# Wu0409/DuPL

Measured on AMD Instinct MI355X. Metric: training img/s at 448^2, VOC dual-student ViT-B/16, phase B step, higher is better.
Workload: dtype f32 storage / accumulation / results; Linear GEMMs (forward, dgrad, wgrad), attention (forward, backward) and the decoder convs as fp32-equivalent f16x3 split products on the f16 MFMA (operands as fp16 hi / lo planes, 3 products per block, fp32 accumulate; error vs fp64 <= the f32 MFMA kernels'); CA

## Files before the change

dupl_amd/csrc/attn_split_bwd.hip:

```cpp
#include "common.h"
#include "../../include/dupl_hip.h"

namespace {

typedef _Float16 h8 __attribute__((ext_vector_type(8)));
typedef _Float16 h4 __attribute__((ext_vector_type(4)));
constexpr float LO_INV = 1.f / DUPL_LO_SCALE;
constexpr int HD = 64, TT = 32;
constexpr int PL = 4096;
constexpr int MAXN = 2048;

#define MFMA16(a, b, c) __builtin_amdgcn_mfma_f32_32x32x16_f16((a), (b), (c), 0, 0, 0)

__device__ __forceinline__ float fast_exp(float x) { return __builtin_amdgcn_exp2f(x * 1.4426950408889634f); }

__device__ __forceinline__ void xcd_remap3(int remap, int& bx, int& by, int& bz) {
    bx = blockIdx.x; by = blockIdx.y; bz = blockIdx.z;
    if (!remap) return;
    const int gx = gridDim.x, gy = gridDim.y;
    const int total = gx * gy * gridDim.z;
    const int L = bx + gx * (by + gy * bz);
    const int q = total >> 3, r = total & 7;
    const int xcd = L & 7, idx = L >> 3;
    const int w = (xcd < r ? xcd * (q + 1) : r * (q + 1) + (xcd - r) * q) + idx;
// ... 67 lines not shown
}

__global__ __launch_bounds__(256) void delta_kernel(const float* __restrict__ out, const float* __restrict__ dout,
                                                    float* __restrict__ delta, int B, int N, int H) {
    const long idx = (long)blockIdx.x * blockDim.x + threadIdx.x;
    const long total = (long)B * N * H;
    if (idx >= total) return;
    const int h = (int)(idx % H);
    const long bn = idx / H;
    const int n = (int)(bn % N), b = (int)(bn / N);
    const float4* o = reinterpret_cast<const float4*>(out + bn * (long)(H * HD) + h * HD);
    const float4* d = reinterpret_cast<const float4*>(dout + bn * (long)(H * HD) + h * HD);
    float s = 0.f;
#pragma unroll
    for (int i = 0; i < HD / 4; ++i) {
        const float4 a = o[i], c = d[i];
        s += (a.x * c.x + a.y * c.y) + (a.z * c.z + a.w * c.w);
    }
    delta[((long)b * H + h) * N + n] = s;
}

__device__ __forceinline__ void attn_bwd16_dq_body(char* __restrict__ smem, const int bx, const int h, const int b,
                                                   const __half* __restrict__ qkv_hi, const __half* __restrict__ qkv_lo,
                                                   const __half* __restrict__ do_hi, const __half* __restrict__ do_lo,
                                                   const float* __restrict__ lse, const float* __restrict__ delta,
                                                   const float* __restrict__ slot, float* __restrict__ dqkv, unsigned int* __restrict__ amax_out, int N, int H,
                                                   float scale) {
    constexpr int STAGE = 6 * PL;
    const int tid = threadIdx.x, lane = tid & 63, wave = tid >> 6, l31 = lane & 31, hf = lane >> 5;
    const int q0 = bx * 128 + wave * 32;
    const int D = H * HD, ld = 3 * D;
    const int qrow = q0 + l31;
// ... 278 lines not shown
    }
    const int bx = w % gx, h = (w / gx) % H, b = w / (gx * H);
    if (role == 0) attn_bwd16_dkv_body<1>(smem, bx, h, b, qkv_hi, qkv_lo, do_hi, do_lo, lse, delta, slot, dqkv, amax_out, N, H, scale);
    else if (role == 1) attn_bwd16_dq_body(smem, bx, h, b, qkv_hi, qkv_lo, do_hi, do_lo, lse, delta, slot, dqkv, amax_out, N, H, scale);
    else attn_bwd16_dkv_body<0>(smem, bx, h, b, qkv_hi, qkv_lo, do_hi, do_lo, lse, delta, slot, dqkv, amax_out, N, H, scale);
}

}

constexpr int g_attnb16_remap = 1;

extern "C" int dupl_attention_bwd16(const void* qkv_hi, const void* qkv_lo, const float* out, const float* dout, const void* do_hi,
                                    const void* do_lo, const float* do_slot, const float* lse, float* delta, float* dqkv, int32_t B,
                                    int32_t N, int32_t H, int32_t hd, float scale, void* amax_out, dupl_stream_t stream) {
    unsigned int* ax = static_cast<unsigned int*>(amax_out);
    if (!qkv_hi || !qkv_lo || !out || !dout || !do_hi || !do_lo || !do_slot || !lse || !delta || !dqkv || B <= 0 || N <= 0 ||
        N > MAXN || H <= 0 || hd != HD)
        return DUPL_ERR_ARG;
    hipStream_t s = (hipStream_t)stream;
    const long total = (long)B * N * H;
    DUPL_LAUNCH(delta_kernel, dim3((unsigned)((total + 255) / 256)), dim3(256), 0, s, out, dout, delta, B, N, H);
    const unsigned blocks = 3u * (unsigned)(((N + 127) / 128) * H * B);
    DUPL_LAUNCH(attn_bwd16_all_kernel, dim3(blocks), dim3(256), 0, s, (const __half*)qkv_hi, (const __half*)qkv_lo,
                       (const __half*)do_hi, (const __half*)do_lo, lse, delta, do_slot, dqkv, ax, N, H, B, scale, g_attnb16_remap);
    return dupl_launch_status();
}
```

dupl_amd/csrc/common.h:

```cpp
#pragma once
#include <hip/hip_runtime.h>
#include <hip/hip_fp16.h>
#include <stdint.h>

#define DUPL_OK 0
#define DUPL_ERR_ARG (-1)
#define DUPL_ERR_LAUNCH (-2)

#define DUPL_WAVE 64


typedef float f32x4 __attribute__((ext_vector_type(4)));
typedef float f32x16 __attribute__((ext_vector_type(16)));

#include <tuple>
#include <utility>
static thread_local int dupl_tl_launch_err = DUPL_OK;

template <typename... KArgs, typename... Args, size_t... I>
static inline hipError_t dupl_launch_impl(void (*kernel)(KArgs...), dim3 grid, dim3 block, size_t shmem, hipStream_t stream,
                                          std::index_sequence<I...>, Args&&... args) {
    std::tuple<KArgs...> vals{static_cast<KArgs>(std::forward<Args>(args))...};
    void* ptrs[sizeof...(KArgs) ? sizeof...(KArgs) : 1] = {static_cast<void*>(&std::get<I>(vals))...};
    return hipLaunchKernel(reinterpret_cast<const void*>(kernel), grid, block, ptrs, shmem, stream);
// ... 21 lines not shown
}
__device__ __forceinline__ float bil_scale(int in, int out, bool align) {
    if (align) return out > 1 ? (float)(in - 1) / (float)(out - 1) : 0.f;
    return (float)in / (float)out;
}

__device__ __forceinline__ float wave_sum(float v) {
#pragma unroll
    for (int o = 32; o > 0; o >>= 1) v += __shfl_xor(v, o, 64);
    return v;
}
__device__ __forceinline__ float wave_max(float v) {
#pragma unroll
    for (int o = 32; o > 0; o >>= 1) v = fmaxf(v, __shfl_xor(v, o, 64));
    return v;
}
__device__ __forceinline__ float wave_min(float v) {
#pragma unroll
    for (int o = 32; o > 0; o >>= 1) v = fminf(v, __shfl_xor(v, o, 64));
    return v;
}
__device__ __forceinline__ double wave_sum_d(double v) {
#pragma unroll
    for (int o = 32; o > 0; o >>= 1) v += __shfl_xor(v, o, 64);
    return v;
}

__device__ __forceinline__ float block_sum(float v, float* red) {
    v = wave_sum(v);
    const int w = threadIdx.x >> 6, l = threadIdx.x & 63, nw = (blockDim.x + 63) >> 6;
// ... 93 lines not shown
```

dupl_amd/csrc/gemm_split.hip:

```cpp
#include "common.h"
#include <type_traits>
#include "../../include/dupl_hip.h"

#ifndef G16_ABL
#define G16_ABL 0
#endif

namespace {

typedef _Float16 h8 __attribute__((ext_vector_type(8)));

constexpr int TBK = 32;
constexpr float LO_INV = 1.f / DUPL_LO_SCALE;

template <bool F1>
__global__ __launch_bounds__(256) void split_kernel(const float* __restrict__ x, __half* __restrict__ hi, __half* __restrict__ lo,
                                                    long n4, float scale) {
    for (long i = (long)blockIdx.x * blockDim.x + threadIdx.x; i < n4; i += (long)gridDim.x * blockDim.x) {
        const float4 v = reinterpret_cast<const float4*>(x)[i];
        __half h[4], l[4];
        if constexpr (F1) {
            split_f32_u(v.x * scale, h[0], l[0]);
            split_f32_u(v.y * scale, h[1], l[1]);
            split_f32_u(v.z * scale, h[2], l[2]);
// ... 1429 lines not shown
    const int g16_f1_big_from = G16_F1_BIG_FROM;
    auto al16 = [](const void* q) { return (reinterpret_cast<uintptr_t>(q) & 15) == 0; };
    if (!al16(d->A_hi) || !al16(d->A_lo) || !al16(d->B_hi) || !al16(d->B_lo)) return DUPL_ERR_ARG;
    if (!d->C && !d->C_hi) return DUPL_ERR_ARG;
    if ((d->C_hi == nullptr) != (d->C_lo == nullptr)) return DUPL_ERR_ARG;
    if ((d->flags & (DUPL_GEMM_STORE_PRE | DUPL_GEMM_MUL_DGELU | DUPL_GEMM_MUL_RELUMASK)) && !d->aux) return DUPL_ERR_ARG;
    if (d->flags & ~(DUPL_GEMM_GELU | DUPL_GEMM_RELU | DUPL_GEMM_STORE_PRE | DUPL_GEMM_ACCUM | DUPL_GEMM_MUL_DGELU |
                     DUPL_GEMM_MUL_RELUMASK))
        return DUPL_ERR_ARG;
    const bool accum = d->flags & DUPL_GEMM_ACCUM;
    if (accum && (!d->C || d->C_hi || d->bias || d->res || d->c_rows)) return DUPL_ERR_ARG;
    if (d->c_rows < 0 || (d->c_rows && (d->flags & (DUPL_GEMM_MUL_DGELU | DUPL_GEMM_MUL_RELUMASK)))) return DUPL_ERR_ARG;
    if (d->amax_out && (accum || d->c_rows || (reinterpret_cast<uintptr_t>(d->amax_out) & 3))) return DUPL_ERR_ARG;
    const bool kmajor = d->a_layout || d->b_layout;
    if (d->fmt < 0 || d->fmt > 1 || d->out_exp < 0 || d->out_exp > 15 || (d->out_exp && d->fmt != 1) ||
        (d->fmt == 1 && !kmajor && (accum || d->amax_out)))
        return DUPL_ERR_ARG;
    hipStream_t s = (hipStream_t)stream;
    int ksplit = 1;
    if (accum) {
        const long tiles = (long)((d->M + 127) / 128) * ((d->N + 127) / 128);
        ksplit = (int)((512 + tiles - 1) / tiles);
        const int maxs = (d->K / TBK + 7) / 8;
        if (ksplit > maxs) ksplit = maxs;
        if (ksplit < 1) ksplit = 1;
        if (d->deterministic) ksplit = 1;
    }
    int tile = g16_tile;
    if (tile == 0) {
        const long b256 = (long)((d->M + 255) / 256) * ((d->N + 127) / 128);
        const long b128 = (long)((d->M + 127) / 128) * ((d->N + 127) / 128) * ksplit;
// ... 41 lines not shown
            else DUPL_LAUNCH((gemm_f16x3_km_kernel<2, 2, 4, 2, 2, false, 2, true, true>), persist_grid(nb21), dim3(512), 0, s, *d, g16_group_ring);
        } else {
            if (d->a_layout || !d->b_layout) return DUPL_ERR_ARG;
            DUPL_LAUNCH((gemm_f16x3_km_kernel<2, 2, 4, 2, 2, false, 0, false, true>), persist_grid(nb21), dim3(512), 0, s, *d, g16_group_ring);
        }
        return dupl_launch_status();
    }
    if (d->fmt == 1) {
        const int nb22 = ((d->M + 255) / 256) * ((d->N + 255) / 256), nb21 = ((d->M + 255) / 256) * ((d->N + 127) / 128);
        int t = (g16_tile == 8 || g16_tile == 12 || g16_tile == 14) ? g16_tile : (nb22 >= g16_f1_big_from ? 8 : 12);
        if (d->K / TBK < 3 && t == 14) t = 12;
        if (t == 8) {
            const int cn = (d->N + 255) / 256, rm = (d->M + 255) / 256, cus = 256;
            const int full = nb22 / cus, tail = nb22 - full * cus;
            const int r_big = full > 0 ? (full * cus) / cn : 0;
            if (g16_tile == 0 && full > 0 && tail > 0 && tail * 10 < cus * 3 && r_big > 0 && r_big < rm && !d->amax_out) {
                const int M1 = r_big * 256;
                dupl_gemm16_desc d1 = *d, d2 = *d;
                d1.M = M1;
                d2.M = d->M - M1;
                auto adv = [&](const void* q, size_t elems, size_t bytes) { return q ? static_cast<const void*>(static_cast<const char*>(q) + elems * bytes) : nullptr; };
                d2.A_hi = adv(d->A_hi, (size_t)M1 * d->lda, 2); d2.A_lo = adv(d->A_lo, (size_t)M1 * d->lda, 2);
                d2.C = (float*)adv(d->C, (size_t)M1 * d->ldc, 4);
                d2.C_hi = (void*)adv(d->C_hi, (size_t)M1 * d->ldo, 2); d2.C_lo = (void*)adv(d->C_lo, (size_t)M1 * d->ldo, 2);
                d2.res = (const float*)adv(d->res, (size_t)M1 * d->ldr, 4);
                d2.aux = (float*)adv(d->aux, (size_t)M1 * d->ldaux, 4);
                if (d->c_rows > 0) {
                    if (d->c_rows <= M1) {
                        d2.c_rows = 0; d2.C = nullptr; d2.aux = nullptr; d2.flags &= ~DUPL_GEMM_STORE_PRE;
                    } else { d1.c_rows = 0; d2.c_rows = d->c_rows - M1; }
                }
// ... 37 lines not shown
```

dupl_amd/csrc/split_prep.hip:

```cpp
#include "common.h"
#include "../../include/dupl_hip.h"

namespace {

__global__ __launch_bounds__(256) void amax_kernel(const float* __restrict__ x, long n4, unsigned int* __restrict__ out) {
    __shared__ float red[4];
    float m = 0.f;
    for (long i = (long)blockIdx.x * blockDim.x + threadIdx.x; i < n4; i += (long)gridDim.x * blockDim.x) {
        const float4 v = reinterpret_cast<const float4*>(x)[i];
        m = fmaxf(m, fmaxf(fmaxf(fabsf(v.x), fabsf(v.y)), fmaxf(fabsf(v.z), fabsf(v.w))));
    }
    m = wave_max(m);
    if ((threadIdx.x & 63) == 0) red[threadIdx.x >> 6] = m;
    __syncthreads();
    if (threadIdx.x == 0) {
        m = fmaxf(fmaxf(red[0], red[1]), fmaxf(red[2], red[3]));
        if (m > 0.f) atomicMax(out, __float_as_uint(m));
    }
}

__device__ __forceinline__ void scale_from_amax(unsigned int bits, int target, float& s, float& inv) {
    const float a = __uint_as_float(bits);
    s = 1.f;
    inv = 1.f;
    if (a > 0.f && a < INFINITY) {
        int e;
        frexpf(a, &e);
        s = ldexpf(1.f, target - e);
        inv = ldexpf(1.f, e - target);
    }
}

template <bool F1 = false>
__device__ __forceinline__ void split_rt_tile(const float* __restrict__ x, const int ld, const int R, const int C, const float s,
                                              __half* __restrict__ hi, __half* __restrict__ lo, __half* __restrict__ hiT,
                                              __half* __restrict__ loT, const int Rp, float* __restrict__ colsum, const int r0,
                                              const int c0, const int Rz = 0) {
    __shared__ unsigned int tile[64][65];
    __shared__ float csum[4][64];
    const int tid = threadIdx.x;
    float4 cs = make_float4(0.f, 0.f, 0.f, 0.f);
#pragma unroll
    for (int i = 0; i < 4; ++i) {
        const int c = tid + 256 * i;
        const int r = c >> 4, cc = (c & 15) << 2;
        float4 v = make_float4(0.f, 0.f, 0.f, 0.f);
        const bool in = r0 + r < R && c0 + cc < C;
        if (in) v = *reinterpret_cast<const float4*>(x + (size_t)(r0 + r) * ld + c0 + cc);
        cs.x += v.x; cs.y += v.y; cs.z += v.z; cs.w += v.w;
        __half h[4], l[4];
        if constexpr (F1) {
            split_f32_u(v.x * s, h[0], l[0]);
            split_f32_u(v.y * s, h[1], l[1]);
            split_f32_u(v.z * s, h[2], l[2]);
            split_f32_u(v.w * s, h[3], l[3]);
        } else {
            split_f32(v.x * s, h[0], l[0]);
            split_f32(v.y * s, h[1], l[1]);
            split_f32(v.z * s, h[2], l[2]);
            split_f32(v.w * s, h[3], l[3]);
        }
        if (hi && c0 + cc < C && r0 + r < (Rz > R ? Rz : R)) {
            *reinterpret_cast<uint2*>(hi + (size_t)(r0 + r) * C + c0 + cc) = *reinterpret_cast<const uint2*>(h);
            *reinterpret_cast<uint2*>(lo + (size_t)(r0 + r) * C + c0 + cc) = *reinterpret_cast<const uint2*>(l);
// ... 27 lines not shown
        const int col = c >> 3, rr = (c & 7) << 3;
        if (c0 + col >= C || r0 + rr >= Rp) continue;
        unsigned int w[8];
#pragma unroll
        for (int j = 0; j < 8; ++j) w[j] = tile[rr + j][col];
        uint4 oh, ol;
        oh.x = (w[0] & 0xffffu) | (w[1] << 16); oh.y = (w[2] & 0xffffu) | (w[3] << 16);
        oh.z = (w[4] & 0xffffu) | (w[5] << 16); oh.w = (w[6] & 0xffffu) | (w[7] << 16);
        ol.x = (w[0] >> 16) | (w[1] & 0xffff0000u); ol.y = (w[2] >> 16) | (w[3] & 0xffff0000u);
        ol.z = (w[4] >> 16) | (w[5] & 0xffff0000u); ol.w = (w[6] >> 16) | (w[7] & 0xffff0000u);
        *reinterpret_cast<uint4*>(hiT + (size_t)(c0 + col) * Rp + r0 + rr) = oh;
        *reinterpret_cast<uint4*>(loT + (size_t)(c0 + col) * Rp + r0 + rr) = ol;
    }
}

template <bool F1>
__global__ __launch_bounds__(256) void split_rt_kernel(const float* __restrict__ x, int ld, int R, int C, float* __restrict__ slot,
                                                       unsigned int* __restrict__ next_bits, __half* __restrict__ hi,
                                                       __half* __restrict__ lo, __half* __restrict__ hiT, __half* __restrict__ loT,
                                                       int Rp, int target, float* __restrict__ colsum, int Rz) {
    float s = 1.f;
    if (slot) {
        float inv;
        scale_from_amax(reinterpret_cast<const unsigned int*>(slot)[2], target, s, inv);
        if (blockIdx.x == 0 && blockIdx.y == 0 && threadIdx.x == 0) {
            slot[0] = s;
            slot[1] = inv;
            if (next_bits) *next_bits = 0u;
        }
    }
    split_rt_tile<F1>(x, ld, R, C, s, hi, lo, hiT, loT, Rp, colsum, blockIdx.y * 64, blockIdx.x * 64, Rz);
}

struct split_multi_args {
    dupl_split_item it[DUPL_SPLIT_MULTI_MAX];
    int first[DUPL_SPLIT_MULTI_MAX + 1];
    int n;
};
__global__ __launch_bounds__(256) void split_rt_multi_kernel(const split_multi_args a) {
    int i = 0;
#pragma unroll 1
    while (i + 1 < a.n && (int)blockIdx.x >= a.first[i + 1]) ++i;
    const dupl_split_item& d = a.it[i];
    const int t = blockIdx.x - a.first[i];
    const int tx = (d.C + 63) / 64;
    split_rt_tile(d.x, d.ld, d.R, d.C, 1.f, (__half*)d.hi, (__half*)d.lo, (__half*)d.hiT, (__half*)d.loT, d.Rp, nullptr,
                  (t / tx) * 64, (t % tx) * 64);
}

}

extern "C" int dupl_split_prepare_multi(const dupl_split_item* items, int32_t n, dupl_stream_t stream) {
    if (!items || n < 1 || n > DUPL_SPLIT_MULTI_MAX) return DUPL_ERR_ARG;
    split_multi_args a;
    a.n = n;
    int total = 0;
    for (int i = 0; i < n; ++i) {
        const dupl_split_item& d = items[i];
        if (!d.x || d.R <= 0 || d.C <= 0 || (d.C & 3) || (d.ld & 3) || d.ld < d.C || (!d.hi && !d.hiT) ||
            ((d.hi == nullptr) != (d.lo == nullptr)) || ((d.hiT == nullptr) != (d.loT == nullptr)) ||
            (d.hiT && (d.Rp < d.R || (d.Rp & 7))) || (reinterpret_cast<uintptr_t>(d.x) & 15))
            return DUPL_ERR_ARG;
        a.it[i] = d;
        a.first[i] = total;
        const int Rt = d.hiT ? d.Rp : d.R;
        total += ((d.C + 63) / 64) * ((Rt + 63) / 64);
    }
    a.first[n] = total;
    DUPL_LAUNCH(split_rt_multi_kernel, dim3((unsigned)total), dim3(256), 0, (hipStream_t)stream, a);
    return dupl_launch_status();
}

extern "C" int dupl_split_prepare(const dupl_split_desc* d, dupl_stream_t stream) {
    if (!d || d->struct_size != sizeof(dupl_split_desc)) return DUPL_ERR_ARG;
    const float* x = d->x;
    const int ld = d->ld, R = d->R, C = d->C, Rp = d->Rp, target_exp = d->target_exp, amax_mode = d->amax_mode;
    float* slot = d->slot;
    void *hi = d->hi, *lo = d->lo, *hiT = d->hiT, *loT = d->loT;
    if (amax_mode < 0 || amax_mode > 2 || (amax_mode && !slot)) return DUPL_ERR_ARG;
    if (d->colsum_accum && d->deterministic) return DUPL_ERR_ARG;
    if (!x || R <= 0 || C <= 0 || (C & 3) || (ld & 3) || ld < C || (!hi && !hiT) || ((hi == nullptr) != (lo == nullptr)) ||
        ((hiT == nullptr) != (loT == nullptr)) || (hiT && (Rp < R || (Rp & 7))) || target_exp < 1 || target_exp > 15)
        return DUPL_ERR_ARG;
    if (d->fmt < 0 || d->fmt > 1 || d->rows_zero_to < 0 || (d->rows_zero_to && (d->rows_zero_to < R || !hi))) return DUPL_ERR_ARG;
    if ((reinterpret_cast<uintptr_t>(x) & 15)) return DUPL_ERR_ARG;
    hipStream_t s = (hipStream_t)stream;
    if (slot && amax_mode != 1) {
        if (ld != C) return DUPL_ERR_ARG;
        if (amax_mode == 2 && hipMemsetAsync(reinterpret_cast<unsigned int*>(slot) + 2, 0, 4, s) != hipSuccess) return DUPL_ERR_LAUNCH;
        const long n4 = (long)R * C / 4;
        long g = (n4 + 2047) / 2048;
        if (g > 256) g = 256;
        if (g < 1) g = 1;
        DUPL_LAUNCH(amax_kernel, dim3((unsigned)g), dim3(256), 0, s, x, n4, reinterpret_cast<unsigned int*>(slot) + 2);
    }
    int Rt = hiT ? Rp : R;
    if (d->rows_zero_to > Rt) Rt = d->rows_zero_to;
    const dim3 grid((C + 63) / 64, (Rt + 63) / 64);
    if (d->fmt == 1)
        DUPL_LAUNCH(split_rt_kernel<true>, grid, dim3(256), 0, s, x, ld, R, C, slot, (unsigned int*)d->next_bits, (__half*)hi,
                           (__half*)lo, (__half*)hiT, (__half*)loT, Rp, target_exp, d->colsum_accum, d->rows_zero_to);
    else
        DUPL_LAUNCH(split_rt_kernel<false>, grid, dim3(256), 0, s, x, ld, R, C, slot, (unsigned int*)d->next_bits, (__half*)hi,
                           (__half*)lo, (__half*)hiT, (__half*)loT, Rp, target_exp, d->colsum_accum, d->rows_zero_to);
    return dupl_launch_status();
}
```

dupl_amd/engine.py:

```python
from __future__ import annotations

import os
from dataclasses import dataclass, field
from typing import Dict, List, Optional, Tuple

import torch

from . import ops

Tensor = torch.Tensor

GEMM_MODE = os.environ.get("DUPL_GEMM", "f16x3")


def set_gemm_mode(mode: str):
    global GEMM_MODE
    assert mode in ("f32", "f16x3"), mode
    GEMM_MODE = mode


@dataclass(frozen=True)
class EncoderConfig:
    embed_dim: int = 768
    depth: int = 12
# ... 55 lines not shown
def param_segment(key: str) -> int:
    if key in ("encoder.pos_embed", "encoder.head.weight", "encoder.head.bias"):
        return SEG_FROZEN
    if key.startswith("encoder."):
        return SEG_NORM if "norm" in key[len("encoder."):] else SEG_BACKBONE
    if key.startswith("decoder."):
        return SEG_DECODER
    return SEG_CLS


FMT1 = os.environ.get("DUPL_FMT1", "1") != "0"
KM_BWD = os.environ.get("DUPL_KM_BWD", "1") != "0"
SK_DGRAD = os.environ.get("DUPL_SK_DGRAD", "1") != "0"
WGRAD_GROUP = os.environ.get("DUPL_WGRAD_GROUP", "1") != "0"

SK_DGRAD_MAX_COLS = 1024
ZERO_WS = os.environ.get("DUPL_ZERO_WS", "1") != "0"
FUSED_PLANES = os.environ.get("DUPL_ADAMW_PLANES", "1") != "0"
MERGED_PASS = int(os.environ.get("DUPL_MERGED_PASS", "16384"))
ATTN_SEGS = int(os.environ.get("DUPL_ATTN_SEGS", "1536"))


class FlatStorage:

    def __init__(self, cfg: EncoderConfig, num_classes: int, n_students: int, device="cpu"):
        self.cfg, self.num_classes, self.n_students = cfg, num_classes, n_students
        shapes = student_param_shapes(cfg, num_classes)
        self.shapes = shapes
        self.layout: Dict[str, Tuple[int, int]] = {}
        self.seg_bounds: List[Tuple[int, int]] = []
# ... 94 lines not shown
        old = self._w16_key[student]
        self._w16_key[student] = key
        self.guard.params_changed(student, rewritten=(old is None or old[0] != key[0] or old[2] != key[2] or old[3] != key[3]),
                                  key=key)

    def w16T(self, student: int, key: str, rows: int):
        ver = self._param_key()
        hit = self._w16T.get((student, key))
        if hit is not None and hit[0] == ver:
            return hit[1]
        w = self.view(student, key).view(rows, -1)
        _, T, _ = ops.split_prepare(w, scaled=False, want_rm=False, want_T=True, rows_pad=rows)
        self._w16T[(student, key)] = (ver, T)
        return T

    def w16T_missing(self, student: int, keys_rows):
        ver = self._param_key()
        out = []
        for key, rows in keys_rows:
            hit = self._w16T.get((student, key))
            if hit is None or hit[0] != ver:
                out.append((key, rows, self.view(student, key).view(rows, -1)))
        return out

    def w16T_put(self, student: int, key: str, T):
        self._w16T[(student, key)] = (self._param_key(), T)

    def w16(self, student: int, key: str, rows: int, fmt1: Optional[bool] = None) -> "ops.W16":
        off, n = self.layout[key]
        base = student * self.student_numel + off
        p = self.data16.data_ptr()
        have = ops.EXP_W if (FMT1 and param_segment(key) == SEG_BACKBONE) else 0
        if fmt1 is None:
            fmt1 = bool(have)
        if bool(have) == bool(fmt1):
            return ops.W16(p + 2 * base, p + 2 * (self.data.numel() + base), rows, n // rows, have)
        assert not fmt1
        ver = self._param_key()
        hit = self._w16F0.get((student, key))
        if hit is None or hit[0] != ver:
            hit = (ver, ops.split16(self.view(student, key).view(rows, -1)))
# ... 217 lines not shown
            self._pos_cache.clear()
            self._pos_version = ver
        key = (h, w)
        if key not in self._pos_cache:
            self._pos_cache[key] = ops.pos_embed_resize(pe, self.cfg.grid, h, w)
        return self._pos_cache[key]

    def mark_grad(self, seg: int):
        self.store.seg_has_grad[self.student][seg] = True

    def w16(self, key: str, rows: int, fmt1: Optional[bool] = None):
        return self.store.w16(self.student, key, rows, fmt1)

    def w16T(self, key: str, rows: int):
        return self.store.w16T(self.student, key, rows)


@dataclass
class BlockSaved:
    x_in: Tensor = None
    mean1: Tensor = None
    rstd1: Tensor = None
    ln1: Tensor = None
    qkv: Tensor = None
    lse: Tensor = None
    att: Tensor = None
    x_mid: Tensor = None
    mean2: Tensor = None
    rstd2: Tensor = None
    ln2: Tensor = None
# ... 442 lines not shown

def _linear_backward16_km(P: StudentParams, dy: Tensor, x16, name: str, dgelu_of: Optional[Tensor] = None,
                          dx_feeds_split: bool = False, wgrads: Optional[list] = None) -> Tensor:
    M, N = dy.shape
    Kp = max(96, (M + 31) // 32 * 32)
    fuse_bias = not ops.deterministic()
    dy16, _, alpha = ops.split_prepare(dy, scaled=True, want_rm=True, want_T=False, fmt1=True, rm_rows=Kp,
                                       colsum_into=P.g[name + ".bias"] if fuse_bias else None)
    gw = P.g[name + ".weight"]
    if wgrads is not None:
        wgrads.append((dy16, x16, gw.view(N, -1), alpha))
    else:
        _lin16(P, dy16, x16, out=gw.view(N, -1), accumulate=True, alpha=alpha, a_kmajor=True, b_kmajor=True, k_pad=Kp)
    if not fuse_bias:
        ops.colsum(dy, P.g[name + ".bias"], accumulate=True)
    W16 = P.w16(name + ".weight", N, True)
    if SK_DGRAD and dgelu_of is None and not dx_feeds_split and not ops.deterministic() and W16.cols <= SK_DGRAD_MAX_COLS:
        dx = ops.zero_workspace(M, W16.cols, dy.device) if ZERO_WS else ops.zeros((M, W16.cols), dy.device)
        _lin16(P, dy16.rows_slice(0, M), W16, out=dx, accumulate=True, alpha=alpha, b_kmajor=True)
        return dx
    dx, _ = _lin16(P, dy16.rows_slice(0, M), W16, alpha=alpha, dgelu_of=dgelu_of, amax_for_next=dx_feeds_split, b_kmajor=True)
    return dx


def _linear_backward16(P: StudentParams, dy: Tensor, x: Tensor, name: str, dgelu_of: Optional[Tensor] = None,
                       has_bias: bool = True, dx_feeds_split: bool = False, xT16=None) -> Tensor:
    M, N = dy.shape
    Mp = (M + 31) // 32 * 32
    fuse_bias = has_bias and not ops.deterministic()
    dy16, dyT16, alpha = ops.split_prepare(dy, scaled=True, want_rm=True, want_T=True, rows_pad=Mp,
# ... 155 lines not shown
```

dupl_amd/ops.py:

```python
from __future__ import annotations

import ctypes
import os
from typing import Optional, Sequence

import numpy as np
import torch

from . import _lib
from ._lib import GemmDesc

Tensor = torch.Tensor


def L():
    return _lib.lib()


_DETERMINISTIC = [os.environ.get("DUPL_DETERMINISTIC", "0") == "1"]


def deterministic() -> bool:
    return _DETERMINISTIC[0]

# ... 145 lines not shown
class _AmaxToken:
    __slots__ = ("word",)


def reserve_amax(device):
    ring = _scale_ring(device)
    if ring[2] is not None:
        return None, None
    tok = _AmaxToken()
    tok.word = ring[0].data_ptr() + 16 * ring[1] + 8
    ring[2] = tok
    return tok.word, tok


def split_prepare(x: Tensor, scaled: bool, want_rm: bool, want_T: bool, rows_pad: int = 0, target_exp: int = 15,
                  colsum_into: Optional[Tensor] = None, fmt1: bool = False, rm_rows: int = 0):
    _chk(x)
    R, C = x.shape
    Rp = rows_pad if rows_pad else (R + 31) // 32 * 32
    rm = None
    if want_rm:
        rm = Split16(torch.empty((2, max(R, rm_rows), C), device=x.device, dtype=torch.float16), 0, fmt=int(fmt1), valid_rows=R)
    T = Split16(torch.empty((2, C, Rp), device=x.device, dtype=torch.float16), 0, fmt=int(fmt1)) if want_T else None
    slot = nxt = rec = None
    amax_mode = 0
    if scaled:
        ring = _scale_ring(x.device)
        pending, ring[2] = ring[2], None
        if pending is not None:
            amax_mode = 1 if getattr(x, "_dupl_amax", None) is pending else 2
        slot, nxt, rec = _scale_slot(x.device)
        assert pending is None or pending.word == slot + 8
    d = _lib.SplitDesc()
    d.x, d.ld, d.R, d.C = x.data_ptr(), x.stride(0), R, C
    d.slot, d.next_bits = slot, nxt
    d.hi, d.lo = (rm.hi, rm.lo) if rm else (None, None)
    d.hiT, d.loT = (T.hi, T.lo) if T else (None, None)
    d.Rp, d.target_exp, d.colsum_accum, d.amax_mode = Rp, target_exp, _p(colsum_into), amax_mode
    d.fmt, d.rows_zero_to = int(fmt1), (rm_rows if (rm is not None and rm_rows > R) else 0)
    d.deterministic = int(deterministic())
    L().dupl_split_prepare(ctypes.byref(d), _stream())
    if scaled:
        for o in (rm, T):
            if o is not None:
                o.planes._dupl_scale = rec
        return rm, T, _Alpha(slot + 4).bind(ring, torch.cuda.current_stream(x.device).cuda_stream)
    return rm, T, None


def split_prepare_multi(items):
    out, descs = [], []
    for x, want_rm, want_T, rows_pad in items:
        _chk(x)
        R, C = x.shape
        Rp = rows_pad if rows_pad else (R + 31) // 32 * 32
        rm = split16_empty(R, C, x.device) if want_rm else None
        T = split16_empty(C, Rp, x.device) if want_T else None
        d = _lib.SplitItem()
        d.x, d.ld, d.R, d.C, d.Rp = x.data_ptr(), x.stride(0), R, C, Rp
        d.hi, d.lo = (rm.hi, rm.lo) if rm else (None, None)
        d.hiT, d.loT = (T.hi, T.lo) if T else (None, None)
        descs.append(d)
        out.append((rm, T))
    for i in range(0, len(descs), _lib.SPLIT_MULTI_MAX):
        chunk = descs[i:i + _lib.SPLIT_MULTI_MAX]
        arr = (_lib.SplitItem * len(chunk))(*chunk)
        L().dupl_split_prepare_multi(ctypes.cast(arr, ctypes.c_void_p), len(chunk), _stream())
    return out


def linear16(x, W: Split16, bias: Optional[Tensor] = None, *, gelu: bool = False, relu: bool = False,
             res: Optional[Tensor] = None, out: Optional[Tensor] = None, store_pre: Optional[Tensor] = None,
             want_f32: bool = True, out16: Optional[Split16] = None, want16: bool = False, device=None,
             alpha: Optional[int] = None, accumulate: bool = False, dgelu_of: Optional[Tensor] = None,
             relumask_of: Optional[Tensor] = None, c_rows: int = 0, amax_for_next: bool = False, out_exp: int = 0,
             a_kmajor: bool = False, b_kmajor: bool = False, k_pad: int = 0, post_exp: int = 0, tuning: Optional[dict] = None):
    M, Ka = (x.cols, x.rows) if a_kmajor else (x.rows, x.cols)
    N, Kb = (W.cols, W.rows) if b_kmajor else (W.rows, W.cols)
    if a_kmajor or b_kmajor:
        K = k_pad if k_pad else max(Ka, Kb)
        assert K % 32 == 0 and K >= 96 and (a_kmajor or Ka == K) and (b_kmajor or Kb == K), (Ka, Kb, K)
    else:
# ... 1 lines not shown
        assert Kb == K and K % 32 == 0
    if dgelu_of is not None or relumask_of is not None:
        assert store_pre is None
        store_pre = dgelu_of if dgelu_of is not None else relumask_of
    dev = device if device is not None else (x.planes.device if isinstance(x, Split16) else x.base.planes.device)
    y = None
    if want_f32 or out is not None:
        y = out if out is not None else torch.empty((c_rows or M, N), device=dev, dtype=torch.float32)
    y16 = out16 if out16 is not None else (split16_empty(M, N, dev, out_exp) if want16 else None)
    d = _lib.Gemm16Desc()
    d.deterministic = int(deterministic())
    xe, we = getattr(x, "exp", 0), getattr(W, "exp", 0)
    xf, wf = getattr(x, "fmt", int(xe > 0)), getattr(W, "fmt", int(we > 0))
    assert xf == wf, f"operand planes in different formats (fmt {xf} / {wf}, exp {xe} / {we})"
    if xf:
        assert (a_kmajor or b_kmajor) or (not accumulate and not amax_for_next)
        assert not (accumulate and b_kmajor and not a_kmajor and deterministic()), "stream-K data gradients use fp32 atomics"
        d.fmt, d.post_scale = 1, 2.0 ** -(xe + we + post_exp)
    if a_kmajor or b_kmajor:
        assert xf == 1, "k-major operands need format 1 planes"
        d.a_layout, d.b_layout = int(a_kmajor), int(b_kmajor)
        d.ka_valid = min(Ka, K) if a_kmajor else 0
        d.kb_valid = min(Kb, K) if b_kmajor else 0
    if y16 is not None:
        assert y16.exp == 0 or xe, "format 1 output planes come from format 1 GEMMs"
        d.out_exp = y16.exp
    d.A_hi, d.A_lo, d.B_hi, d.B_lo = x.hi, x.lo, W.hi, W.lo
    d.C = _p(y)
    d.C_hi, d.C_lo = (y16.hi, y16.lo) if y16 is not None else (None, None)
    d.bias, d.res, d.aux = _p(bias), _p(res), _p(store_pre)
    d.M, d.N, d.K = M, N, K
# ... 215 lines not shown
    for i, (row0, B, N, out, need_lse, b_f32) in enumerate(segs):
        bf = b_f32 or B
        assert out is not None or out16 is not None
        if out is not None:
            assert out.shape == (bf * N, H * hd) and out.is_contiguous()
        lse = torch.empty((bf, H, N), device=dev, dtype=torch.float32) if need_lse else None
        lses.append(lse)
        arr[i].row0, arr[i].B, arr[i].N, arr[i].B_f32 = int(row0), int(B), int(N), int(b_f32)
        arr[i].out, arr[i].lse = _p(out), _p(lse)
    L().dupl_attention_fwd16_segs(qkv16.hi, qkv16.lo, out16.hi if out16 is not None else None,
                                   out16.lo if out16 is not None else None, ctypes.cast(arr, ctypes.c_void_p), len(segs), H, hd,
                                   float(scale), out16.exp if out16 is not None else 0, _stream())
    return lses


def attention_bwd16(qkv16, out: Tensor, dout: Tensor, lse: Tensor, B: int, N: int, H: int, hd: int, scale: float,
                    amax_for_next: bool = False) -> Tensor:
    assert hd == 64 and N <= 2048 and qkv16.rows == B * N
    dev = out.device
    dout = dout.contiguous()
    do16, _, alpha = split_prepare(dout, scaled=True, want_rm=True, want_T=False, target_exp=4)
    alpha.check()
    delta = torch.empty((B, H, N), device=dev, dtype=torch.float32)
    dqkv = torch.empty((B * N, 3 * H * hd), device=dev, dtype=torch.float32)
    word, tok = reserve_amax(dev) if amax_for_next else (None, None)
    L().dupl_attention_bwd16(qkv16.hi, qkv16.lo, out.data_ptr(), dout.data_ptr(), do16.hi, do16.lo, int(alpha) - 4, lse.data_ptr(),
                             delta.data_ptr(), dqkv.data_ptr(), B, N, H, hd, float(scale), word, _stream())
    if tok is not None:
        dqkv._dupl_amax = tok
    return dqkv


def attention_bwd(qkv: Tensor, out: Tensor, dout: Tensor, lse: Tensor, B: int, N: int, H: int, hd: int, scale: float) -> Tensor:
    dqkv = torch.empty_like(qkv)
    delta = torch.empty((B, H, N), device=qkv.device, dtype=torch.float32)
    L().dupl_attention_bwd(qkv.data_ptr(), out.data_ptr(), dout.data_ptr(), lse.data_ptr(), delta.data_ptr(),
                           dqkv.data_ptr(), B, N, H, hd, scale, _stream())
    return dqkv


def patch_im2row(x: Tensor, P: int) -> Tensor:
# ... 379 lines not shown
```

include/dupl_hip.h:

```cpp
#ifndef DUPL_HIP_H
#define DUPL_HIP_H

#include <stdint.h>

#ifdef __cplusplus
extern "C" {
#endif

typedef void* dupl_stream_t;

int dupl_abi_version(void);
int dupl_build_digest(char* out, int32_t cap);

#define DUPL_LOSS_SUMS_FLOATS 136
#define DUPL_GEMM_A_MCONTIG 1
#define DUPL_GEMM_B_NCONTIG 2
#define DUPL_GEMM_GELU 4
#define DUPL_GEMM_ACCUM 8
#define DUPL_GEMM_MUL_DGELU 16
#define DUPL_GEMM_RELU 32
#define DUPL_GEMM_MUL_RELUMASK 64
#define DUPL_GEMM_ABS 128
#define DUPL_GEMM_STORE_PRE 256
typedef struct dupl_gemm_desc {
// ... 49 lines not shown
int dupl_gemm_f16x3_group(const dupl_gemm16_desc* descs, int32_t n, dupl_stream_t stream);
int dupl_split_f16x2(const float* x, void* hi, void* lo, int64_t n, dupl_stream_t stream);
int dupl_split_f16x2b(const float* x, void* hi, void* lo, int64_t n, int32_t scale_exp, dupl_stream_t stream);
typedef struct dupl_split_desc {
    uint32_t struct_size;
    int32_t ld, R, C;
    const float* x;
    float* slot; void* next_bits;
    void* hi; void* lo; void* hiT; void* loT;
    int32_t Rp, target_exp;
    float* colsum_accum;
    int32_t amax_mode, fmt, rows_zero_to;
    int32_t deterministic;
} dupl_split_desc;
int dupl_split_prepare(const dupl_split_desc* d, dupl_stream_t stream);
#define DUPL_SPLIT_MULTI_MAX 16
typedef struct dupl_split_item {
    const float* x; void* hi; void* lo; void* hiT; void* loT;
    int32_t ld, R, C, Rp;
} dupl_split_item;
int dupl_split_prepare_multi(const dupl_split_item* items, int32_t n, dupl_stream_t stream);
typedef struct dupl_bound_desc {
    int64_t offset;
    int32_t rows, cols;
} dupl_bound_desc;
int dupl_param_bounds(const float* base, const dupl_bound_desc* table_dev, int32_t n, float* out, dupl_stream_t stream);

int dupl_layernorm_fwd(const float* x, const float* gamma, const float* beta, float* y,
                       float* mean, float* rstd, int64_t rows, int32_t D, float eps, dupl_stream_t s);
int dupl_layernorm_fwd16(const float* x, const float* gamma, const float* beta, float* y, void* y_hi, void* y_lo, float* mean,
                         float* rstd, int64_t rows, int32_t D, float eps, int64_t f32_rows, int32_t plane_exp, dupl_stream_t s);
int dupl_layernorm_bwd_blocks(int64_t rows, int32_t rows_per_wave);
int dupl_layernorm_bwd(const float* dy, const float* x, const float* gamma, const float* mean,
                       const float* rstd, const float* dres, float* dx, float* dgamma, float* dbeta,
                       int64_t rows, int32_t D, void* amax_out, float* partials, int64_t partial_rows, int32_t rows_per_wave,
                       float* dy_clear, int32_t deterministic, dupl_stream_t s);
// ... 188 lines not shown
```

Measured before the change: 76.54.

## Fuse attention delta into dout split and add pre-transposed fp16 dgrad weights

The attention backward delta (rowwise dot of out and dout per head) is now computed inside the split-prepare kernel that already reads dout, so the separate delta kernel and its extra read of dout are skipped. Separately, mlp.fc2 data-gradient GEMMs now use cached, pre-transposed fmt1 weight planes, prepared in groups across blocks, and the non-k-major fmt1 path now accepts amax output. This trades a separate launch and memory pass for extra shuffles in the split kernel, plus more cached weight planes and some loosened argument checks.

Result: no change. 77.19 (median of 6 runs) (+0.8%).

```diff
diff --git a/dupl_amd/csrc/attn_split_bwd.hip b/dupl_amd/csrc/attn_split_bwd.hip
--- a/dupl_amd/csrc/attn_split_bwd.hip
+++ b/dupl_amd/csrc/attn_split_bwd.hip
@@ -105,8 +105,7 @@
     float s = 0.f;
 #pragma unroll
     for (int i = 0; i < HD / 4; ++i) {
-        const float4 a = o[i], c = d[i];
-        s += (a.x * c.x + a.y * c.y) + (a.z * c.z + a.w * c.w);
+        s = __fadd_rn(s, delta_dot4(o[i], d[i]));
     }
     delta[((long)b * H + h) * N + n] = s;
 }
@@ -415,12 +414,12 @@
                                     const void* do_lo, const float* do_slot, const float* lse, float* delta, float* dqkv, int32_t B,
                                     int32_t N, int32_t H, int32_t hd, float scale, void* amax_out, dupl_stream_t stream) {
     unsigned int* ax = static_cast<unsigned int*>(amax_out);
-    if (!qkv_hi || !qkv_lo || !out || !dout || !do_hi || !do_lo || !do_slot || !lse || !delta || !dqkv || B <= 0 || N <= 0 ||
+    if (!qkv_hi || !qkv_lo || !dout || !do_hi || !do_lo || !do_slot || !lse || !delta || !dqkv || B <= 0 || N <= 0 ||
         N > MAXN || H <= 0 || hd != HD)
         return DUPL_ERR_ARG;
     hipStream_t s = (hipStream_t)stream;
     const long total = (long)B * N * H;
-    DUPL_LAUNCH(delta_kernel, dim3((unsigned)((total + 255) / 256)), dim3(256), 0, s, out, dout, delta, B, N, H);
+    if (out) DUPL_LAUNCH(delta_kernel, dim3((unsigned)((total + 255) / 256)), dim3(256), 0, s, out, dout, delta, B, N, H);
     const unsigned blocks = 3u * (unsigned)(((N + 127) / 128) * H * B);
     DUPL_LAUNCH(attn_bwd16_all_kernel, dim3(blocks), dim3(256), 0, s, (const __half*)qkv_hi, (const __half*)qkv_lo,
                        (const __half*)do_hi, (const __half*)do_lo, lse, delta, do_slot, dqkv, ax, N, H, B, scale, g_attnb16_remap);
diff --git a/dupl_amd/csrc/common.h b/dupl_amd/csrc/common.h
--- a/dupl_amd/csrc/common.h
+++ b/dupl_amd/csrc/common.h
@@ -59,6 +59,9 @@
 #pragma unroll
     for (int o = 32; o > 0; o >>= 1) v = fmaxf(v, __shfl_xor(v, o, 64));
     return v;
+}
+__device__ __forceinline__ float delta_dot4(const float4 a, const float4 c) {
+    return __fadd_rn(__fmaf_rn(a.x, c.x, __fmul_rn(a.y, c.y)), __fmaf_rn(a.z, c.z, __fmul_rn(a.w, c.w)));
 }
 __device__ __forceinline__ float wave_min(float v) {
 #pragma unroll
diff --git a/dupl_amd/csrc/gemm_split.hip b/dupl_amd/csrc/gemm_split.hip
--- a/dupl_amd/csrc/gemm_split.hip
+++ b/dupl_amd/csrc/gemm_split.hip
@@ -1467,7 +1467,7 @@
     if (d->amax_out && (accum || d->c_rows || (reinterpret_cast<uintptr_t>(d->amax_out) & 3))) return DUPL_ERR_ARG;
     const bool kmajor = d->a_layout || d->b_layout;
     if (d->fmt < 0 || d->fmt > 1 || d->out_exp < 0 || d->out_exp > 15 || (d->out_exp && d->fmt != 1) ||
-        (d->fmt == 1 && !kmajor && (accum || d->amax_out)))
+        (d->fmt == 1 && !kmajor && accum))
         return DUPL_ERR_ARG;
     hipStream_t s = (hipStream_t)stream;
     int ksplit = 1;
@@ -1539,7 +1539,7 @@
             const int cn = (d->N + 255) / 256, rm = (d->M + 255) / 256, cus = 256;
             const int full = nb22 / cus, tail = nb22 - full * cus;
             const int r_big = full > 0 ? (full * cus) / cn : 0;
-            if (g16_tile == 0 && full > 0 && tail > 0 && tail * 10 < cus * 3 && r_big > 0 && r_big < rm && !d->amax_out) {
+            if (g16_tile == 0 && full > 0 && tail > 0 && tail * 10 < cus * 3 && r_big > 0 && r_big < rm) {
                 const int M1 = r_big * 256;
                 dupl_gemm16_desc d1 = *d, d2 = *d;
                 d1.M = M1;
diff --git a/dupl_amd/csrc/split_prep.hip b/dupl_amd/csrc/split_prep.hip
--- a/dupl_amd/csrc/split_prep.hip
+++ b/dupl_amd/csrc/split_prep.hip
@@ -31,11 +31,12 @@
     }
 }
 
-template <bool F1 = false>
+template <bool F1 = false, bool DL = false>
 __device__ __forceinline__ void split_rt_tile(const float* __restrict__ x, const int ld, const int R, const int C, const float s,
                                               __half* __restrict__ hi, __half* __restrict__ lo, __half* __restrict__ hiT,
                                               __half* __restrict__ loT, const int Rp, float* __restrict__ colsum, const int r0,
-                                              const int c0, const int Rz = 0) {
+                                              const int c0, const int Rz = 0, const float* __restrict__ dot_o = nullptr,
+                                              float* __restrict__ delta = nullptr, const int seq = 1) {
     __shared__ unsigned int tile[64][65];
     __shared__ float csum[4][64];
     const int tid = threadIdx.x;
@@ -48,6 +49,18 @@
         const bool in = r0 + r < R && c0 + cc < C;
         if (in) v = *reinterpret_cast<const float4*>(x + (size_t)(r0 + r) * ld + c0 + cc);
         cs.x += v.x; cs.y += v.y; cs.z += v.z; cs.w += v.w;
+        if constexpr (DL) {
+            float4 o = make_float4(0.f, 0.f, 0.f, 0.f);
+            if (in) o = *reinterpret_cast<const float4*>(dot_o + (size_t)(r0 + r) * ld + c0 + cc);
+            const float part = delta_dot4(o, v);
+            float dsum = 0.f;
+#pragma unroll
+            for (int k = 0; k < 16; ++k) dsum = __fadd_rn(dsum, __shfl(part, (tid & 48) | k, 64));
+            if ((tid & 15) == 0 && r0 + r < R) {
+                const int gr = r0 + r, b = gr / seq, n = gr - b * seq;
+                delta[((size_t)b * (C >> 6) + (c0 >> 6)) * seq + n] = dsum;
+            }
+        }
         __half h[4], l[4];
         if constexpr (F1) {
             split_f32_u(v.x * s, h[0], l[0]);
@@ -105,11 +118,13 @@
     }
 }
 
-template <bool F1>
+template <bool F1, bool DL = false>
 __global__ __launch_bounds__(256) void split_rt_kernel(const float* __restrict__ x, int ld, int R, int C, float* __restrict__ slot,
                                                        unsigned int* __restrict__ next_bits, __half* __restrict__ hi,
                                                        __half* __restrict__ lo, __half* __restrict__ hiT, __half* __restrict__ loT,
-                                                       int Rp, int target, float* __restrict__ colsum, int Rz) {
+                                                       int Rp, int target, float* __restrict__ colsum, int Rz,
+                                                       const float* __restrict__ dot_o = nullptr, float* __restrict__ delta = nullptr,
+                                                       int seq = 1) {
     float s = 1.f;
     if (slot) {
         float inv;
@@ -120,12 +135,13 @@
             if (next_bits) *next_bits = 0u;
         }
     }
-    split_rt_tile<F1>(x, ld, R, C, s, hi, lo, hiT, loT, Rp, colsum, blockIdx.y * 64, blockIdx.x * 64, Rz);
+    split_rt_tile<F1, DL>(x, ld, R, C, s, hi, lo, hiT, loT, Rp, colsum, blockIdx.y * 64, blockIdx.x * 64, Rz, dot_o, delta, seq);
 }
 
 struct split_multi_args {
     dupl_split_item it[DUPL_SPLIT_MULTI_MAX];
     int first[DUPL_SPLIT_MULTI_MAX + 1];
+    int exp[DUPL_SPLIT_MULTI_MAX];
     int n;
 };
 __global__ __launch_bounds__(256) void split_rt_multi_kernel(const split_multi_args a) {
@@ -135,19 +151,26 @@
     const dupl_split_item& d = a.it[i];
     const int t = blockIdx.x - a.first[i];
     const int tx = (d.C + 63) / 64;
-    split_rt_tile(d.x, d.ld, d.R, d.C, 1.f, (__half*)d.hi, (__half*)d.lo, (__half*)d.hiT, (__half*)d.loT, d.Rp, nullptr,
-                  (t / tx) * 64, (t % tx) * 64);
-}
-
-}
-
-extern "C" int dupl_split_prepare_multi(const dupl_split_item* items, int32_t n, dupl_stream_t stream) {
+    const int e = a.exp[i];
+    if (e > 0)
+        split_rt_tile<true>(d.x, d.ld, d.R, d.C, ldexpf(1.f, e), (__half*)d.hi, (__half*)d.lo, (__half*)d.hiT, (__half*)d.loT, d.Rp,
+                            nullptr, (t / tx) * 64, (t % tx) * 64);
+    else
+        split_rt_tile(d.x, d.ld, d.R, d.C, 1.f, (__half*)d.hi, (__half*)d.lo, (__half*)d.hiT, (__half*)d.loT, d.Rp, nullptr,
+                      (t / tx) * 64, (t % tx) * 64);
+}
+
+}
+
+extern "C" int dupl_split_prepare_multi_fmt(const dupl_split_item* items, const int32_t* scale_exp, int32_t n, dupl_stream_t stream) {
     if (!items || n < 1 || n > DUPL_SPLIT_MULTI_MAX) return DUPL_ERR_ARG;
     split_multi_args a;
     a.n = n;
     int total = 0;
     for (int i = 0; i < n; ++i) {
         const dupl_split_item& d = items[i];
+        a.exp[i] = scale_exp ? scale_exp[i] : 0;
+        if (a.exp[i] < 0 || a.exp[i] > 15) return DUPL_ERR_ARG;
         if (!d.x || d.R <= 0 || d.C <= 0 || (d.C & 3) || (d.ld & 3) || d.ld < d.C || (!d.hi && !d.hiT) ||
             ((d.hi == nullptr) != (d.lo == nullptr)) || ((d.hiT == nullptr) != (d.loT == nullptr)) ||
             (d.hiT && (d.Rp < d.R || (d.Rp & 7))) || (reinterpret_cast<uintptr_t>(d.x) & 15))
@@ -162,7 +185,11 @@
     return dupl_launch_status();
 }
 
-extern "C" int dupl_split_prepare(const dupl_split_desc* d, dupl_stream_t stream) {
+extern "C" int dupl_split_prepare_multi(const dupl_split_item* items, int32_t n, dupl_stream_t stream) {
+    return dupl_split_prepare_multi_fmt(items, nullptr, n, stream);
+}
+
+static int split_prepare_impl(const dupl_split_desc* d, const float* dot_o, float* delta, int seq, dupl_stream_t stream) {
     if (!d || d->struct_size != sizeof(dupl_split_desc)) return DUPL_ERR_ARG;
     const float* x = d->x;
     const int ld = d->ld, R = d->R, C = d->C, Rp = d->Rp, target_exp = d->target_exp, amax_mode = d->amax_mode;
@@ -188,11 +215,26 @@
     int Rt = hiT ? Rp : R;
     if (d->rows_zero_to > Rt) Rt = d->rows_zero_to;
     const dim3 grid((C + 63) / 64, (Rt + 63) / 64);
+    if (delta) {
+        if (!dot_o || seq <= 0 || (R % seq) || (C & 63) || (reinterpret_cast<uintptr_t>(dot_o) & 15) || d->fmt != 0) return DUPL_ERR_ARG;
+        DUPL_LAUNCH((split_rt_kernel<false, true>), grid, dim3(256), 0, s, x, ld, R, C, slot, (unsigned int*)d->next_bits, (__half*)hi,
+                           (__half*)lo, (__half*)hiT, (__half*)loT, Rp, target_exp, d->colsum_accum, d->rows_zero_to, dot_o, delta, seq);
+        return dupl_launch_status();
+    }
     if (d->fmt == 1)
         DUPL_LAUNCH(split_rt_kernel<true>, grid, dim3(256), 0, s, x, ld, R, C, slot, (unsigned int*)d->next_bits, (__half*)hi,
-                           (__half*)lo, (__half*)hiT, (__half*)loT, Rp, target_exp, d->colsum_accum, d->rows_zero_to);
+                           (__half*)lo, (__half*)hiT, (__half*)loT, Rp, target_exp, d->colsum_accum, d->rows_zero_to, nullptr, nullptr, 1);
     else
         DUPL_LAUNCH(split_rt_kernel<false>, grid, dim3(256), 0, s, x, ld, R, C, slot, (unsigned int*)d->next_bits, (__half*)hi,
-                           (__half*)lo, (__half*)hiT, (__half*)loT, Rp, target_exp, d->colsum_accum, d->rows_zero_to);
+                           (__half*)lo, (__half*)hiT, (__half*)loT, Rp, target_exp, d->colsum_accum, d->rows_zero_to, nullptr, nullptr, 1);
     return dupl_launch_status();
 }
+
+extern "C" int dupl_split_prepare(const dupl_split_desc* d, dupl_stream_t stream) {
+    return split_prepare_impl(d, nullptr, nullptr, 1, stream);
+}
+
+extern "C" int dupl_split_prepare_delta(const dupl_split_desc* d, const float* out, float* delta, int32_t seq, dupl_stream_t stream) {
+    if (!out || !delta) return DUPL_ERR_ARG;
+    return split_prepare_impl(d, out, delta, seq, stream);
+}
diff --git a/dupl_amd/engine.py b/dupl_amd/engine.py
--- a/dupl_amd/engine.py
+++ b/dupl_amd/engine.py
@@ -93,6 +93,7 @@
 SK_DGRAD = os.environ.get("DUPL_SK_DGRAD", "1") != "0"
 WGRAD_GROUP = os.environ.get("DUPL_WGRAD_GROUP", "1") != "0"
 
+DGRAD_FWD_TILE = tuple(t for t in os.environ.get("DUPL_DGRAD_FWD_TILE", "mlp.fc2").split(",") if t)
 SK_DGRAD_MAX_COLS = 1024
 ZERO_WS = os.environ.get("DUPL_ZERO_WS", "1") != "0"
 FUSED_PLANES = os.environ.get("DUPL_ADAMW_PLANES", "1") != "0"
@@ -217,17 +218,30 @@
         self._w16T[(student, key)] = (ver, T)
         return T
 
-    def w16T_missing(self, student: int, keys_rows):
+    def w16T_missing(self, student: int, keys_rows, fmt1: bool = False):
         ver = self._param_key()
         out = []
         for key, rows in keys_rows:
-            hit = self._w16T.get((student, key))
+            hit = self._w16T.get((student, key, 1) if fmt1 else (student, key))
             if hit is None or hit[0] != ver:
                 out.append((key, rows, self.view(student, key).view(rows, -1)))
         return out
 
-    def w16T_put(self, student: int, key: str, T):
-        self._w16T[(student, key)] = (self._param_key(), T)
+    def w16T_put(self, student: int, key: str, T, fmt1: bool = False):
+        self._w16T[(student, key, 1) if fmt1 else (student, key)] = (self._param_key(), T)
+
+    def w16T_f1(self, student: int, key: str, rows: int, group=()):
+        assert FMT1 and param_segment(key) == SEG_BACKBONE and rows % 32 == 0
+        ver = self._param_key()
+        hit = self._w16T.get((student, key, 1))
+        if hit is not None and hit[0] == ver:
+            return hit[1]
+        want = [(key, rows)] + [kr for kr in group if kr[0] != key]
+        stale = self.w16T_missing(student, want, fmt1=True)
+        out = ops.split_prepare_multi([(w, False, True, r, ops.EXP_W) for _, r, w in stale])
+        for (k, _, _), (_, T) in zip(stale, out):
+            self.w16T_put(student, k, T, fmt1=True)
+        return self._w16T[(student, key, 1)][1]
 
     def w16(self, student: int, key: str, rows: int, fmt1: Optional[bool] = None) -> "ops.W16":
         off, n = self.layout[key]
@@ -475,6 +489,9 @@
 
     def w16T(self, key: str, rows: int):
         return self.store.w16T(self.student, key, rows)
+
+    def w16T_f1(self, key: str, rows: int, group=()):
+        return self.store.w16T_f1(self.student, key, rows, group)
 
 
 @dataclass
@@ -947,6 +964,13 @@
         _lin16(P, dy16, x16, out=gw.view(N, -1), accumulate=True, alpha=alpha, a_kmajor=True, b_kmajor=True, k_pad=Kp)
     if not fuse_bias:
         ops.colsum(dy, P.g[name + ".bias"], accumulate=True)
+    site = name.split(".", 3)[-1]
+    if site in DGRAD_FWD_TILE and N % 32 == 0 and (dgelu_of is not None or dx_feeds_split or ops.deterministic()):
+        group = [(f"encoder.blocks.{j}.{st_}.weight", P.w[f"encoder.blocks.{j}.{st_}.weight"].shape[0])
+                 for st_ in DGRAD_FWD_TILE for j in range(P.cfg.depth)]
+        WT16 = P.w16T_f1(name + ".weight", N, group)
+        dx, _ = _lin16(P, dy16.rows_slice(0, M), WT16, alpha=alpha, dgelu_of=dgelu_of, amax_for_next=dx_feeds_split)
+        return dx
     W16 = P.w16(name + ".weight", N, True)
     if SK_DGRAD and dgelu_of is None and not dx_feeds_split and not ops.deterministic() and W16.cols <= SK_DGRAD_MAX_COLS:
         dx = ops.zero_workspace(M, W16.cols, dy.device) if ZERO_WS else ops.zeros((M, W16.cols), dy.device)
diff --git a/dupl_amd/ops.py b/dupl_amd/ops.py
--- a/dupl_amd/ops.py
+++ b/dupl_amd/ops.py
@@ -183,7 +183,7 @@
 
 
 def split_prepare(x: Tensor, scaled: bool, want_rm: bool, want_T: bool, rows_pad: int = 0, target_exp: int = 15,
-                  colsum_into: Optional[Tensor] = None, fmt1: bool = False, rm_rows: int = 0):
+                  colsum_into: Optional[Tensor] = None, fmt1: bool = False, rm_rows: int = 0, delta_of=None):
     _chk(x)
     R, C = x.shape
     Rp = rows_pad if rows_pad else (R + 31) // 32 * 32
@@ -208,7 +208,13 @@
     d.Rp, d.target_exp, d.colsum_accum, d.amax_mode = Rp, target_exp, _p(colsum_into), amax_mode
     d.fmt, d.rows_zero_to = int(fmt1), (rm_rows if (rm is not None and rm_rows > R) else 0)
     d.deterministic = int(deterministic())
-    L().dupl_split_prepare(ctypes.byref(d), _stream())
+    if delta_of is not None:
+        o_, delta, seq = delta_of
+        assert not fmt1 and C % 64 == 0 and x.stride(0) == C and o_.shape == x.shape and o_.is_contiguous() and R % seq == 0
+        assert delta.is_contiguous() and delta.numel() == R * (C // 64) and delta.dtype == torch.float32 == o_.dtype
+        L().dupl_split_prepare_delta(ctypes.byref(d), o_.data_ptr(), delta.data_ptr(), int(seq), _stream())
+    else:
+        L().dupl_split_prepare(ctypes.byref(d), _stream())
     if scaled:
         for o in (rm, T):
             if o is not None:
@@ -218,13 +224,15 @@
 
 
 def split_prepare_multi(items):
-    out, descs = [], []
-    for x, want_rm, want_T, rows_pad in items:
+    out, descs, exps = [], [], []
+    for x, want_rm, want_T, rows_pad, *rest in items:
         _chk(x)
         R, C = x.shape
+        e = int(rest[0]) if rest else 0
         Rp = rows_pad if rows_pad else (R + 31) // 32 * 32
-        rm = split16_empty(R, C, x.device) if want_rm else None
-        T = split16_empty(C, Rp, x.device) if want_T else None
+        rm = split16_empty(R, C, x.device, e) if want_rm else None
+        T = split16_empty(C, Rp, x.device, e) if want_T else None
+        exps.append(e)
         d = _lib.SplitItem()
         d.x, d.ld, d.R, d.C, d.Rp = x.data_ptr(), x.stride(0), R, C, Rp
         d.hi, d.lo = (rm.hi, rm.lo) if rm else (None, None)
@@ -234,7 +242,8 @@
     for i in range(0, len(descs), _lib.SPLIT_MULTI_MAX):
         chunk = descs[i:i + _lib.SPLIT_MULTI_MAX]
         arr = (_lib.SplitItem * len(chunk))(*chunk)
-        L().dupl_split_prepare_multi(ctypes.cast(arr, ctypes.c_void_p), len(chunk), _stream())
+        ex = (ctypes.c_int32 * len(chunk))(*exps[i:i + _lib.SPLIT_MULTI_MAX])
+        L().dupl_split_prepare_multi_fmt(ctypes.cast(arr, ctypes.c_void_p), ctypes.cast(ex, ctypes.c_void_p), len(chunk), _stream())
     return out
 
 
@@ -266,7 +275,7 @@
     xf, wf = getattr(x, "fmt", int(xe > 0)), getattr(W, "fmt", int(we > 0))
     assert xf == wf, f"operand planes in different formats (fmt {xf} / {wf}, exp {xe} / {we})"
     if xf:
-        assert (a_kmajor or b_kmajor) or (not accumulate and not amax_for_next)
+        assert (a_kmajor or b_kmajor) or not accumulate
         assert not (accumulate and b_kmajor and not a_kmajor and deterministic()), "stream-K data gradients use fp32 atomics"
         d.fmt, d.post_scale = 1, 2.0 ** -(xe + we + post_exp)
     if a_kmajor or b_kmajor:
@@ -512,17 +521,22 @@
     return lses
 
 
+FUSED_DELTA = _os.environ.get("DUPL_FUSED_DELTA", "1") != "0"
+
+
 def attention_bwd16(qkv16, out: Tensor, dout: Tensor, lse: Tensor, B: int, N: int, H: int, hd: int, scale: float,
                     amax_for_next: bool = False) -> Tensor:
     assert hd == 64 and N <= 2048 and qkv16.rows == B * N
     dev = out.device
     dout = dout.contiguous()
-    do16, _, alpha = split_prepare(dout, scaled=True, want_rm=True, want_T=False, target_exp=4)
+    delta = torch.empty((B, H, N), device=dev, dtype=torch.float32)
+    fused = FUSED_DELTA and out.is_contiguous() and out.shape == dout.shape
+    do16, _, alpha = split_prepare(dout, scaled=True, want_rm=True, want_T=False, target_exp=4,
+                                   delta_of=(out, delta, N) if fused else None)
     alpha.check()
-    delta = torch.empty((B, H, N), device=dev, dtype=torch.float32)
     dqkv = torch.empty((B * N, 3 * H * hd), device=dev, dtype=torch.float32)
     word, tok = reserve_amax(dev) if amax_for_next else (None, None)
-    L().dupl_attention_bwd16(qkv16.hi, qkv16.lo, out.data_ptr(), dout.data_ptr(), do16.hi, do16.lo, int(alpha) - 4, lse.data_ptr(),
+    L().dupl_attention_bwd16(qkv16.hi, qkv16.lo, None if fused else out.data_ptr(), dout.data_ptr(), do16.hi, do16.lo, int(alpha) - 4, lse.data_ptr(),
                              delta.data_ptr(), dqkv.data_ptr(), B, N, H, hd, float(scale), word, _stream())
     if tok is not None:
         dqkv._dupl_amax = tok
diff --git a/include/dupl_hip.h b/include/dupl_hip.h
--- a/include/dupl_hip.h
+++ b/include/dupl_hip.h
@@ -87,12 +87,14 @@
     int32_t deterministic;
 } dupl_split_desc;
 int dupl_split_prepare(const dupl_split_desc* d, dupl_stream_t stream);
+int dupl_split_prepare_delta(const dupl_split_desc* d, const float* out, float* delta, int32_t seq, dupl_stream_t stream);
 #define DUPL_SPLIT_MULTI_MAX 16
 typedef struct dupl_split_item {
     const float* x; void* hi; void* lo; void* hiT; void* loT;
     int32_t ld, R, C, Rp;
 } dupl_split_item;
 int dupl_split_prepare_multi(const dupl_split_item* items, int32_t n, dupl_stream_t stream);
+int dupl_split_prepare_multi_fmt(const dupl_split_item* items, const int32_t* scale_exp, int32_t n, dupl_stream_t stream);
 typedef struct dupl_bound_desc {
     int64_t offset;
     int32_t rows, cols;
```
